# MatchaChoco010/toy-cpu-pathtracing

Measured on AMD Instinct MI355X. Metric: Msamples/sec (whole node), scene3 MIS/Sobol 1920x1080, higher is better.
Workload: dtype f32; 1 GPU; scene3 1920x1080 mis+sobol, 1024-spp job, 1024 sample indices per step (BASELINE configs[1]); parallelism=single-gpu

## Files before the change

### toy-cpu-pathtracing_amd/csrc/api.cpp

```cpp
#include <cstring>

#include "api_internal.hpp"

using namespace pt;

static thread_local std::string g_err;
bool pt::g_debug_unlocked = false;
int pt::fail(int code, const std::string& msg) { g_err = msg; return code; }

static const uint32_t CIE_CMF_BITS[470 * 4] = {
#include "cie_cmf.inc"
};
void pt::cie_cmf4(float out[470 * 4]) { std::memcpy(out, CIE_CMF_BITS, sizeof(CIE_CMF_BITS)); }

int pt::get_launch_ctx(const mi355pt_scene* sc, uint32_t seed, LaunchCtx** out, int* slot) {
    if (sc->ctx && sc->ctx->device != sc->impl.device) {
        delete sc->ctx; sc->ctx = nullptr;
    }
    if (!sc->ctx) {
        LaunchCtx* lc = new LaunchCtx();
        lc->device = sc->impl.device;
        HIP_TRY(hipMalloc((void**)&lc->d_hash, sizeof(uint64_t) * HASH_TABLE_DIMS));
        HIP_TRY(hipMalloc((void**)&lc->d_counters, sizeof(unsigned) * CTX_RING));
        HIP_TRY(hipMalloc((void**)&lc->d_stats, sizeof(DevStats) * CTX_RING));
// ... 88 lines not shown
    int rc;
    LaunchCtx* lc; int slot;
    if ((rc = get_launch_ctx(s, p->seed, &lc, &slot))) return rc;
    if (lc->device != s->impl.device) return fail(MI355PT_E_DEVICE, "launch context and scene live on different devices");
    const bool want_stats = stats && p->collect_stats;
    int& waves = aov ? lc->aov_waves[aov_kind] : lc->waves[want_stats ? 1 : 0][p->sampler & 1u][p->strategy < 3u ? p->strategy : 0u];
    if (!waves) waves = aov ? query_resident_waves_aov((uint32_t)aov_kind, s->impl.features)
                            : query_resident_waves(select_kernel(false, want_stats, s->impl.features, p->sampler, p->strategy));
    const DevCamera dc = make_camera(cam);
    LaunchPlan plan = d_list ? plan_launch_tiles(cam, p, s_begin, s_end, waves, n_list) : plan_launch(cam, p, s_begin, s_end, waves, aov);
    DevParams& dp = plan.params;
    if (d_list) set_tile_list(dp, d_list);
    dp.stats_mode = p->collect_stats;
    return timed_launch(lc, slot, stream, stats, want_stats || aov, [&](unsigned* d_counter, DevStats* d_stats) {
        if ((rc = grow_device_buffer(&lc->d_partial, &lc->partial_bytes, plan.partial_floats * sizeof(float), stream))) return rc;
        const KernelKey key = select_kernel(d_list != nullptr, want_stats, s->impl.features, p->sampler, p->strategy);
        if ((rc = grow_device_buffer(&lc->d_defer, &lc->defer_bytes, aov ? (size_t)0 : query_defer_bytes_per_wave(key) * (size_t)plan.grid, stream))) return rc;
        if (aov) HIP_TRY(launch_aov((uint32_t)aov_kind, s->impl.dev, dc, dp, illuminant_lut, lc->d_hash, d_accum, d_counter, stats ? d_stats : nullptr,
                                    s->impl.features, plan.grid, stream));
        else {
            DevScene dev = s->impl.dev;
            dev.cam_lists = use_camera_lists(key, dp.block_log2, camera_lists_enabled()) ? 1u : 0u;
            dev.queue_stage = use_queue_staging(key, queue_staging_enabled()) ? 1u : 0u;
            HIP_TRY(launch_pt(key, dev, dc, dp, plan.n_tiles,
                              lc->d_hash, d_accum, lc->d_partial, d_counter, d_list ? nullptr : d_stats, plan.grid, stream, pout, lc->d_defer));
        }
        return (int)MI355PT_OK;
    });
}

int pt::launch_ranges(const mi355pt_scene* s, const mi355pt_camera* cam, const mi355pt_params* p, uint32_t s_begin, uint32_t s_end, float* d_accum,
                      hipStream_t stream, mi355pt_stats* stats, const uint32_t* d_list, uint32_t n_list, const PathOut& pout, int aov_kind,
                      uint32_t illuminant_lut) {
    return for_each_launch_range(p->sampler, stats != nullptr, s_begin, s_end, [&](uint32_t b, uint32_t e) {
        return launch_range(s, cam, p, b, e, d_accum, stream, stats, pout, aov_kind, illuminant_lut, d_list, n_list);
    });
}

int pt::render_accum_range(const mi355pt_scene* s, const mi355pt_camera* cam, const mi355pt_params* p, uint32_t s_begin, uint32_t s_end,
                           float* d_accum, void* hip_stream, mi355pt_stats* stats, const PathOut& pout, int aov_kind, uint32_t illuminant_lut) {
    const bool aov = aov_kind >= 0;
    int rc = check_args(s, cam, p, aov);
    if (rc) return rc;
    if (!d_accum || s_end > p->spp || s_begin >= s_end) return fail(MI355PT_E_INVALID, "bad sample range or null accumulator");
    if (aov) {
        if (aov_kind > MI355PT_AOV_SHADING_NORMAL) return fail(MI355PT_E_INVALID, "unknown AOV kind");
// ... 97 lines not shown
```

### toy-cpu-pathtracing_amd/csrc/launch_plan.hpp

```cpp
#pragma once
#include <algorithm>
#include <cmath>
#include <cstddef>
#include <cstdint>
#include <cstdlib>

#include "../../include/mi355pt.h"
#include "layout.hpp"

namespace pt {

struct V3 { float x, y, z; };
inline V3 cross3(V3 a, V3 b) { return {a.y * b.z - b.y * a.z, a.z * b.x - b.z * a.x, a.x * b.y - b.x * a.y}; }
inline V3 norm3(V3 a) { float r = 1.0f / std::sqrt((a.x * a.x) + (a.y * a.y) + (a.z * a.z)); return {a.x * r, a.y * r, a.z * r}; }

inline uint32_t log2_int(uint32_t v) { return v == 0 ? 0 : 31 - (uint32_t)__builtin_clz(v); }
inline uint32_t round_up_pow2(uint32_t v) { return v <= 1 ? 1 : 1u << (32 - __builtin_clz(v - 1)); }

inline uint32_t shard_tile_count(uint32_t width, uint32_t height, uint32_t shard_index, uint32_t shard_count) {
    const uint32_t total = ((width + 7) / 8) * ((height + 7) / 8);
    const uint32_t cnt = shard_count ? shard_count : 1u, idx = shard_count ? shard_index : 0u;
    return total > idx ? (total - idx + cnt - 1) / cnt : 0u;
}

// ... 133 lines not shown
inline constexpr uint32_t FEATURE_SETS[] = {PT_FOR_EACH_SET(PT_SET_ENTRY, PT_SET_ENTRY)};
inline constexpr uint32_t PLAIN_SETS[] = {PT_FOR_EACH_PLAIN_SET(PT_SET_ENTRY)};
inline constexpr uint32_t CC_SETS[] = {PT_FOR_EACH_CC_SET(PT_SET_ENTRY)};
#undef PT_SET_ENTRY
inline uint32_t pick_features(uint32_t feat) {
    for (uint32_t s : FEATURE_SETS) if ((feat & ~s) == 0u) return s;
    return FEAT_ALL;
}
struct KernelKey { bool tiles, stats; uint32_t mode, set; };
inline KernelKey select_kernel(bool tiles, bool stats, uint32_t feat, uint32_t sampler, uint32_t strategy) {
    if (stats) return KernelKey{tiles, true, MODE_GENERIC, (feat & (FEAT_CC | FEAT_EMTEX)) == 0u ? FEAT_STD & ~FEAT_CC : FEAT_ALL};
    const uint32_t mode = sampler == MI355PT_SAMPLER_SOBOL && strategy == MI355PT_STRATEGY_MIS ? MODE_MIS_SOBOL
                        : sampler == MI355PT_SAMPLER_SOBOL && strategy == MI355PT_STRATEGY_NEE ? MODE_NEE_SOBOL
                        : strategy == MI355PT_STRATEGY_PT ? MODE_PT : MODE_GENERIC;
    return KernelKey{tiles, false, mode, pick_features(feat)};
}

inline bool use_camera_lists(const KernelKey& key, uint32_t block_log2, bool enabled) { return enabled && !key.stats && block_log2 <= 3u; }
inline bool camera_lists_enabled() { const char* e = getenv("MI355PT_NO_CAMERA_LISTS"); return !(e && e[0] != '\0' && !(e[0] == '0' && e[1] == '\0')); }

inline bool use_queue_staging(const KernelKey& key, bool enabled) { return enabled && !key.stats; }
inline bool queue_staging_enabled() { const char* e = getenv("MI355PT_NO_QUEUE_STAGING"); return !(e && e[0] != '\0' && !(e[0] == '0' && e[1] == '\0')); }

}
```

### toy-cpu-pathtracing_amd/csrc/layout.hpp

```cpp
#pragma once
#include <stddef.h>
#include <stdint.h>

#if defined(__HIPCC__)
#define PT_HD __host__ __device__
#else
#define PT_HD
#endif

namespace pt {

#ifndef PT_STACK_DEPTH
#define PT_STACK_DEPTH 24
#endif
constexpr int STACK_DEPTH = PT_STACK_DEPTH;
constexpr int MAX_LEAF_TRIS = 4;
constexpr int MAX_BUILD_DEPTH = 22;
constexpr int HASH_TABLE_DIMS = 136;

struct alignas(16) DevNode {
    float bx[4];
    float by[4];
    float bz[4];
    int32_t child[2];
// ... 138 lines not shown
    const DevTriLocal* tris_local;
    const DevTri* tris_render;
    float tri_shift[3]; uint32_t tris_are_local;
    float shared_mw[3]; uint32_t pad_mw;
    const DevInstance* instances;
    const DevMaterial* materials;
    const DevLight* lights;
    const DevLightTri* light_tris;
    const float* light_uvs;
    const float* luts;
    const float* cmf;
    const float* rgb2spec;
    const float* z_nodes;
    const uint32_t* texels;
    const DevTexture* textures;
    const float* cc_albedo;
    uint32_t n_nodes, n_tris, n_lights, n_materials;
    int32_t root;
    int32_t root4;
    uint32_t n_nodes4;
    uint32_t cam_lists;
    const DevEnv* envs;
    uint32_t n_envs;
    uint32_t queue_stage;
};

struct DevCamera {
    float s[3], u[3], f[3];
    float tan_half_fov, aspect;
    uint32_t width, height;
};

struct DevParams {
    uint32_t spp, seed, max_depth, strategy, sampler;
    float exposure;
    uint32_t log2_spp, n_base4_digits;
    uint32_t sample_begin, sample_end;
    uint32_t shard_index, shard_count;
    uint32_t tiles_x, tiles_y;
    uint32_t n_work;
    uint32_t chunks, chunk_size;
    uint32_t block_log2;
    uint32_t sample_prefix_digits;
    uint32_t stats_mode;
    uint32_t albedo_lut;
    float rr_gate;
    float xyz_to_rgb[9];
// ... 21 lines not shown
```

### toy-cpu-pathtracing_amd/csrc/pt_kernel.hpp

```cpp
#pragma once
#include <hip/hip_runtime.h>

#include "launch.hpp"
#include "launch_plan.hpp"
#include "layout.hpp"
#include "pt_device.hpp"
#include "pt_path.hpp"
#include "tail_queue_plan.hpp"
#define PT_CAM_UNIFORM(v) ((uint32_t)__builtin_amdgcn_readfirstlane((int)(v)))
#include "camera_candidates.hpp"

namespace pt {

constexpr uint32_t CAM_LIST_NONE = 0xffffffffu;

#ifndef PT_MIN_WAVES_CC
#define PT_MIN_WAVES_CC 3
#endif
#ifndef PT_MIN_WAVES
#define PT_MIN_WAVES 4
#endif
struct LaneJob { uint32_t px, py, s_cur, s_end; bool valid; };
template <typename TileOf>
PT_DEV LaneJob lane_job_at(uint32_t work, uint32_t lane, const DevCamera& cam, const DevParams& prm, TileOf tile_of) {
// ... 47 lines not shown
constexpr uint32_t DEFER_F4 = 8u;
constexpr uint32_t defer_classes_of(uint32_t FEAT, uint32_t MODE) {
    if (!merged_traversal_of(FEAT, MODE)) return 0u;
    if ((FEAT & FEAT_CC) != 0u) return (1u << MT_CLEARCOAT) | (1u << (MT_CLEARCOAT | 8u));
    if ((FEAT & FEAT_TEX) != 0u) return 0xff00u;
    return 0u;
}
template <uint32_t FEAT, uint32_t MODE> constexpr uint32_t defer_classes() { return defer_classes_of(FEAT, MODE); }
#ifndef PT_TAILQ
#define PT_TAILQ 1
#endif
#ifndef PT_TAILQ_MIN
#define PT_TAILQ_MIN 64
#endif
constexpr bool tail_queue_of(uint32_t FEAT, uint32_t MODE) { return PT_TAILQ != 0 && merged_traversal_of(FEAT, MODE); }
template <uint32_t FEAT, uint32_t MODE> constexpr bool tail_queue() { return tail_queue_of(FEAT, MODE); }
constexpr uint32_t QUEUE_RING = (PT_TAILQ != 0) ? 256u : DEFER_RING;
constexpr uint32_t QUEUE_MAX = (PT_TAILQ != 0) ? 2u : 1u;
static_assert(PT_TAILQ == 0 || QUEUE_RING == 256u, "the tail queue's entry index keeps the queue number in bit 8");
constexpr uint32_t TQ_F4 = 5u;
#ifndef PT_TAILQ_RING1
#define PT_TAILQ_RING1 128u
#endif
constexpr size_t queue_bytes_per_wave(bool STATS, uint32_t FEAT, uint32_t MODE) {
    if (!STATS && tail_queue_of(FEAT, MODE)) return (size_t)16u * TQ_F4 * ((FEAT & FEAT_CC) != 0u ? QUEUE_MAX * QUEUE_RING : PT_TAILQ_RING1);
    return defer_classes_of(FEAT, MODE) != 0u ? (size_t)16u * DEFER_F4 * DEFER_RING : (size_t)0;
}
template <uint32_t FEAT> constexpr int kernel_min_waves() {
    if ((FEAT & FEAT_CC) == 0u) return PT_MIN_WAVES;
    if (FEAT != (FEAT_CC | FEAT_TEX)) return 4;
    return PT_MIN_WAVES_CC;
}
template <bool STATS, uint32_t FEAT, uint32_t MODE = MODE_GENERIC>
__global__ __launch_bounds__(64, kernel_min_waves<FEAT>()) void pt_kernel(DevScene sc, DevCamera cam, DevParams prm_in, const uint64_t* __restrict__ dim_hash_tab,
                                                float* __restrict__ accum, float* __restrict__ partial, unsigned* __restrict__ work_counter,
                                                DevStats* __restrict__ stats, PathOut pout, float4* __restrict__ defer_buf) {
#define PT_LANE_JOB lane_job
#include "pt_kernel_body.inc"
#undef PT_LANE_JOB
}

PT_DEV void item_sobol_prefixes(SamplerCtx& sctx, const DevParams& prm, const LaneJob& job0, uint32_t lane, uint32_t* s_hi, uint32_t* s_p6, uint32_t n_dims) {
    const uint32_t blk_log2 = prm.block_log2;
    const uint32_t s_prefix = prm.sample_prefix_digits;
    const uint32_t hi_first_w = sobol_hi_first(prm.log2_spp, blk_log2) - s_prefix, hi_shift_w = 2u * hi_first_w - (prm.log2_spp & 1u);
    if (prm.sampler == 1u && hi_first_w < prm.n_base4_digits && hi_first_w >= 3u &&
        2u * prm.n_base4_digits - (prm.log2_spp & 1u) <= hi_shift_w + 27u) {
        sctx.hi_first = sobol_hi_first(prm.log2_spp, blk_log2) - s_prefix;
// ... 28 lines not shown
```

### toy-cpu-pathtracing_amd/csrc/pt_kernel_body.inc

```
    __shared__ __attribute__((aligned(16))) uint32_t s_stack[STACK_DEPTH * 64];
#ifndef PT_FILM_PIX
#define PT_FILM_PIX 64
#endif
    __shared__ float s_film[PT_FILM_PIX * 3];
    __shared__ uint32_t s_hi[SOBOL_HI_DIMS];
    __shared__ uint32_t s_p6[SOBOL_HI_DIMS];
    __shared__ unsigned s_work;
    constexpr bool PARK = (FEAT & FEAT_CC) != 0u && kernel_min_waves<FEAT>() <= 3;
    __shared__ float s_park[PARK ? 8 * 64 : 1];
    __shared__ uint8_t s_perm[96];
    __shared__ uint32_t s_ring[ANY_RING];
    __shared__ uint32_t s_occl[2];
    __shared__ uint32_t s_pair[64];
    const AnyLds any_lds{s_ring, s_occl, s_pair};
    __shared__ unsigned long long s_best[64];
    const ClosestLds closest_lds{s_ring, s_best, s_pair};
    __shared__ uint32_t s_infl[2];
    const PairLds pair_lds{s_ring, s_best, s_occl, s_pair, s_infl};
    constexpr bool CAMLIST = !STATS && tail_queue<FEAT, MODE>();
    __shared__ uint32_t s_cand[CAMLIST ? CAM_LIST_CAP : 1u];
    DevParams prm = prm_in;
    if constexpr (MODE == MODE_MIS_SOBOL) { prm.strategy = 2u; prm.sampler = 1u; }
    if constexpr (MODE == MODE_NEE_SOBOL) { prm.strategy = 1u; prm.sampler = 1u; }
    if constexpr (MODE == MODE_PT) prm.strategy = 0u;
// ... 65 lines not shown
        if (lane < PT_FILM_PIX) { s_film[3 * lane] = 0.0f; s_film[3 * lane + 1] = 0.0f; s_film[3 * lane + 2] = 0.0f; }
        __syncthreads();
        const uint32_t n_s = job0.s_end > job0.s_cur ? job0.s_end - job0.s_cur : 0u;
        const uint32_t pool_size = n_s << (2u * blk_log2);
        uint32_t pool_next = 0u;
        uint32_t my_pix = lane;
        Path P{};
        park(P);
        bool active = false;
        constexpr bool MERGED = merged_traversal<FEAT, MODE>();
        ShadowReq sh{};
        bool dying = false, susp = false;
        CarryState carry{0ull};
        constexpr bool TAILQ = !STATS && tail_queue<FEAT, MODE>();
        constexpr uint32_t DEFER = TAILQ ? 0u : defer_classes<FEAT, MODE>();
        float4* const q_base = (DEFER != 0u || TAILQ) ? defer_buf + (size_t)blockIdx.x * (queue_bytes_per_wave(STATS, FEAT, MODE) / 16u) : nullptr;
        uint32_t q_head = 0u, q_tail = 0u;
        uint32_t q_count = 0u, q2_count = 0u;
        constexpr uint32_t TQ_CLASSES = (TAILQ && (FEAT & FEAT_CC) != 0u) ? ((1u << MT_CLEARCOAT) | (1u << (MT_CLEARCOAT | 8u))) : 0u;
        constexpr uint32_t QR = (TQ_CLASSES != 0u) ? QUEUE_RING : PT_TAILQ_RING1;
        constexpr bool STAGE = TAILQ && TQ_CLASSES == 0u;
        static_assert(STACK_DEPTH * 64 >= (int)(TQ_STAGE_SLOTS * TQ_F4 * 4u) && TQ_STAGE_SLOTS == 64u, "a pass's worth of staged tail-queue records fits the traversal stack's LDS");
        float4* const s_stage = (float4*)s_stack;
        while (true) {
            unsigned long long ts0 = 0, ts1 = 0, ts2 = 0, ts3 = 0, ts4 = 0, tsa = 0, tsb = 0;
            uint32_t bsdf_classes = 0u;
            if (STATS) ts0 = __builtin_amdgcn_s_memtime();
            bool popped = false;
            uint32_t pop_e = 0u;
            const unsigned long long m_needy = __ballot(!active);
            if (m_needy != 0ull && pool_next < pool_size) {
                const uint32_t idx = pool_next + rank_below(m_needy);
                if (!active && idx < pool_size) {
                    const uint32_t pix = idx & ((1u << (2u * blk_log2)) - 1u);
                    const uint32_t px = job0.px + (pix & blk_mask), py = job0.py + (pix >> blk_log2);
                    const uint32_t smp_i = job0.s_cur + (idx >> (2u * blk_log2));
                    const bool valid = px < cam.width && py < cam.height;
                    if (valid) { active = true; my_pix = pix; regen_path<STATS>(P, sctx, cam, px, py, smp_i, st); }
                }
                pool_next = min(pool_next + (uint32_t)__popcll(m_needy), pool_size);
            }
            if (!__any(active)) {
                if (pool_next >= pool_size && q_tail == q_head && (q_count | q2_count) == 0u) break;
                if (!((DEFER != 0u || TAILQ) && pool_next >= pool_size)) continue;
            }
            if (STATS) { ts1 = __builtin_amdgcn_s_memtime(); if (lane == 0) st.w[4]++; if (active) st.w[5]++; }
            Hit hit{};
            bool got = false;
            const bool canonical = STATS && prm.stats_mode == 1u;
            if (canonical) { if (active) got = trace_closest<STATS>(sc, P.ro, P.rd, 3.402823466e+38f, stack, hit, st); }
            else if constexpr (MERGED) {
                bool occluded = false;
                if (STATS && sh.on) st.w[6]++;
                bool cam_ray = false;
                if constexpr (CAMLIST) cam_ray = cam_n != CAM_LIST_NONE && active && !dying && P.from_camera && P.depth == 0u;
                if (!CAMLIST || __ballot((active && !dying && !popped && !cam_ray) || sh.on) != 0ull) {
                    PT_PRIO_TRAV_ENTER;
                    trace_pair_coop<STATS>(sc, P.ro, P.rd, active && !dying && !popped && !cam_ray, sh.o, sh.d, sh.t, sh.on, stack, lane, pair_lds, hit, got, occluded, st, &carry, susp, &susp);
                    PT_PRIO_TRAV_EXIT;
                }
                if constexpr (CAMLIST) {
                    if (__ballot(cam_ray) != 0ull) {
                        const RaySetup rs = setup_ray(P.rd);
                        const f3 o2 = tri_origin(sc, P.ro);
                        unsigned long long key = (0x7f7fffffull << 32) | 0xffffffffull;
                        for (uint32_t i = 0u; i < cam_n; ++i) {
// ... 76 lines not shown
                const uint32_t fl = __float_as_uint(b.y);
                Q.smp.morton = __float_as_uint(a.x); Q.smp.dimension = __float_as_uint(a.y); Q.smp.rkey_lo = __float_as_uint(a.z); Q.smp.rkey_hi = __float_as_uint(a.w);
                Q.wl.lam0 = b.x; Q.wl.term = (fl & 1u) != 0u; Q.from_camera = (fl & 2u) != 0u; Q.prev_spec = (fl & 4u) != 0u; Q.depth = (fl >> 3) & 1023u; pix = fl >> 16;
                Q.T[0] = b.z; Q.T[1] = b.w; Q.T[2] = c.x; Q.T[3] = c.y; Q.L[0] = c.z; Q.L[1] = c.w; Q.L[2] = d.x; Q.L[3] = d.y;
                Q.rd = mk3(d.z, d.w, e4.x); Q.ro = mk3(0.0f, 0.0f, 0.0f);
                Q.pf[0] = e4.y; Q.pf[1] = e4.z; Q.pf[2] = e4.w; Q.pf[3] = f.x; Q.p_pdf = f.y; Q.prev_pos = mk3(f.z, f.w, g.x);
                h.t = g.y; h.b0 = g.z; h.b1 = g.w; h.b2 = h4.x; h.tri = __float_as_uint(h4.y); h.mclass = __float_as_uint(h4.z);
            };
            auto finish_path = [&]() {
                if (pout.L != nullptr) {
                    const uint32_t px = job0.px + (my_pix & blk_mask), py = job0.py + (my_pix >> blk_log2);
                    const uint32_t tile_k = (work / prm.chunks) >> (6u - 2u * blk_log2);
                    const uint32_t smp_i = P.smp.morton & ((1u << prm.log2_spp) - 1u);
                    sample_log(P, pout, ((size_t)tile_k * 64u + ((py & 7u) * 8u + (px & 7u))) * pout.n_s + (smp_i - pout.s_base));
                }
                float r, g, b;
                film_rgb(P, sc, prm, r, g, b);
                atomicAdd(&s_film[3 * my_pix], r); atomicAdd(&s_film[3 * my_pix + 1], g); atomicAdd(&s_film[3 * my_pix + 2], b);
            };
            if constexpr (TAILQ) {
                bool end_path = dying;
                const bool front = active && !dying && !susp;
                unpark(P);
                {
                    ShadeCtx C0;
                    C0.cont = false;
                    if (front) end_path = shade_vertex_head<STATS, FEAT, 1>(P, sc, prm, sctx, got, hit, sh, st, tsa, C0);
                }
                dying = false;
                const bool go_on = front && !end_path;
                const bool cls2 = TQ_CLASSES != 0u && ((TQ_CLASSES >> (hit.mclass & 31u)) & 1u) != 0u;
                const unsigned long long m_on1 = __ballot(go_on && !cls2), m_on2 = TQ_CLASSES != 0u ? __ballot(go_on && cls2) : 0ull;
                uint32_t n_on1 = 0u;
                bool stage = false;
                if constexpr (STAGE) {
                    n_on1 = (uint32_t)__popcll(m_on1);
                    stage = sc.queue_stage != 0u && tq_stage_pushes(q_count, n_on1, pool_next >= pool_size, (uint32_t)PT_TAILQ_MIN);
                }
                if ((m_on1 | m_on2) != 0ull) {
                    if (go_on) {
                        if (STAGE && stage) tq_put(s_stage + tq_stage_push_index(rank_below(m_on1)), TQ_STAGE_SLOTS, P, hit, my_pix);
                        else {
                            const uint32_t e = cls2 ? QUEUE_RING + tq_push_slot(q2_count, rank_below(m_on2)) : tq_push_slot(q_count, rank_below(m_on1));
                            tq_store(e, P, hit, my_pix);
                        }
                        active = false;
                    }
                    q_count += (uint32_t)__popcll(m_on1); q2_count += (uint32_t)__popcll(m_on2);
                    __builtin_amdgcn_fence(__ATOMIC_RELEASE, "workgroup");
                }
                if (active && end_path) { finish_path(); active = false; }
                park(P, false);
                if (STATS) ts3 = ts4 = __builtin_amdgcn_s_memtime();
                const bool draining = pool_next >= pool_size;
                if (tq_pass_due(q_count, q2_count, draining, TQ_CLASSES != 0u, (uint32_t)PT_TAILQ_MIN)) {
                    const unsigned long long m_free = __ballot(!active);
                    const uint32_t n_free = (uint32_t)__popcll(m_free), r = rank_below(m_free);
                    const TqTake tk = tq_pass_take(q_count, q2_count, n_free, draining, TQ_CLASSES != 0u, (uint32_t)PT_TAILQ_MIN);
                    const uint32_t n2 = tk.n2, n1 = tk.n1;
                    const bool take2 = !active && r < n2, take1 = !active && !take2 && r - n2 < n1;
                    const bool take = take1 || take2;
                    const uint32_t e = take2 ? QUEUE_RING + tq_pop_slot(q2_count, n2, r) : tq_pop_slot(q_count, n1, r - n2);
                    TqStagePop sp{0u, false, 0u};
                    if constexpr (STAGE) sp = tq_stage_pop(stage ? q_count - n_on1 : q_count, stage ? n_on1 : 0u, n1, r - n2);
                    q2_count -= n2; q_count -= n1;
                    bool ep = false;
                    if constexpr ((FEAT & FEAT_CC) != 0u) {
                        ShadeCtx C;
                        shade_ctx_idle_cc(C);
                        if (take) {
                            __builtin_amdgcn_fence(__ATOMIC_ACQUIRE, "workgroup");
                            tq_load(e, P, hit, my_pix);
                            active = true;
                            shade_vertex_head<STATS, FEAT, 2>(P, sc, prm, sctx, true, hit, sh, st, tsa, C);
                        }
// ... 140 lines not shown
```

### toy-cpu-pathtracing_amd/csrc/pt_path.hpp

```cpp
#pragma once
#include "launch.hpp"
#include "pt_device.hpp"
#include "pt_ggx.hpp"

namespace pt {

constexpr float RAY_EPS = 1e-5f;
constexpr float SHADOW_EPS = 1e-4f;

struct Frame { f3 t, b, n; };
PT_DEV f3 to_local(const Frame& f, f3 v) { return mk3(dot(f.t, v), dot(f.b, v), dot(f.n, v)); }
PT_DEV f3 to_world(const Frame& f, f3 v) { return f.t * v.x + f.b * v.y + f.n * v.z; }
PT_DEV Frame shading_frame(f3 shading_normal, f3 tangent) {
    Frame f;
    f.n = normalize(shading_normal);
    f.b = normalize(cross(normalize(f.n), tangent));
    f.t = normalize(cross(f.b, f.n));
    return f;
}
#ifndef PT_EXACT_DIV
#define PT_EXACT_DIV 0
#endif
#ifndef PT_FRAME_INVERSE
#define PT_FRAME_INVERSE 2
// ... 218 lines not shown
    float dx = (2.0f * fx / (float)cam.width - 1.0f) * cam.aspect * cam.tan_half_fov;
    float dy = (1.0f - 2.0f * fy / (float)cam.height) * cam.tan_half_fov;
    f3 dc = normalize(mk3(dx, dy, -1.0f));
    f3 s = mk3(cam.s[0], cam.s[1], cam.s[2]), uu = mk3(cam.u[0], cam.u[1], cam.u[2]), ff = mk3(cam.f[0], cam.f[1], cam.f[2]);
    rd = normalize(s * dc.x + uu * dc.y + (-ff) * dc.z);
    ro = mk3(0, 0, 0) + rd * RAY_EPS;
#pragma unroll
    for (int i = 0; i < 4; ++i) { T[i] = 1.0f; L[i] = 0.0f; }
    from_camera = true; depth = 0; need_new = false;
    if (STATS) st.samples++;
    (void)need_new;
}

PT_DEV f3 camera_ray_dir(const DevCamera& cam, uint32_t px, uint32_t py, f2 uv) {
    float fx = (float)px + (uv.x * 1.0f - 1.0f * 0.5f) + 0.5f;
    float fy = (float)py + (uv.y * 1.0f - 1.0f * 0.5f) + 0.5f;
    float dx = (2.0f * fx / (float)cam.width - 1.0f) * cam.aspect * cam.tan_half_fov;
    float dy = (1.0f - 2.0f * fy / (float)cam.height) * cam.tan_half_fov;
    f3 dc = normalize(mk3(dx, dy, -1.0f));
    f3 s = mk3(cam.s[0], cam.s[1], cam.s[2]), uu = mk3(cam.u[0], cam.u[1], cam.u[2]), ff = mk3(cam.f[0], cam.f[1], cam.f[2]);
    return normalize(s * dc.x + uu * dc.y + (-ff) * dc.z);
}

struct ShadeCtx {
    Surface sf; const DevMaterial* mat; uint32_t mtype;
    Frame fr, fw, nf, nfw; f3 wo, wo_nm, ng_t; float geo_wo, uc; f2 uv;
    bool is_diel, rough_diel, cont;
    float d_alpha;
    bool need_cc; float cc_alpha_c, cc_r0c, cc_thick, cc_metallic, cc_rough_b, cc_fc; uint64_t mc_key;
};

PT_DEV void shade_ctx_idle_cc(ShadeCtx& C) {
    C.cont = false; C.need_cc = false; C.cc_fc = 0.0f; C.cc_alpha_c = 0.0f; C.cc_r0c = 0.0f; C.wo_nm = mk3(0, 0, 1); C.mc_key = 0ull;
}

template <bool STATS, uint32_t FEAT, int PHASE = 0>
PT_DEV bool shade_vertex_head(Path& P, const DevScene& sc, const DevParams& prm, const SamplerCtx& sctx, bool got, const Hit& hit, ShadowReq& sh,
                           StatCounters& st, unsigned long long& tsa, ShadeCtx& C) {
    Sampler& smp = P.smp; Wl& wl = P.wl; float* T = P.T; float* L = P.L; f3& ro = P.ro; f3& rd = P.rd;
    bool& from_camera = P.from_camera; bool& prev_spec = P.prev_spec; float* pf = P.pf; float& p_pdf = P.p_pdf; f3& prev_pos = P.prev_pos;
    uint32_t& depth = P.depth;
    bool end_path = false;
    bool& do_shadow = sh.on; f3& sh_o = sh.o; f3& sh_d = sh.d; float& sh_t = sh.t; float* sh_c = sh.c;
    do_shadow = false;

    if (PHASE != 2 && !got) {
// ... 26 lines not shown
                    }
                    for (uint32_t li = 0; li < sc.n_lights; ++li) {
                        DevLight lt = sc.lights[li];
                        if (lt.kind != LK_ENV) continue;
                        const DevMaterial* lm = sc.materials + lt.material;
                        float ph[4];
                        DevSpectrum ls = load_spectrum(&lm->color);
                        eval_spectrum<false, (FEAT & FEAT_EMTEX) != 0, (FEAT & FEAT_EMTEX) != 0>(sc, ls, wl, f2{0.5f, 0.5f}, ph, st);
                        float sum = 0.0f;
#pragma unroll
                        for (int i = 0; i < 4; ++i) sum += (ph[i] * lm->intensity_avg) * lt.area_sum;
                        const float probability = inf_sum == 0.0f ? 0.0f : (sum / 4.0f) / inf_sum;
                        light_pdf += probability * env_pdf(sc.envs[lt.first_tri], rd);
                    }
                }
                float w = balance_heuristic(p_pdf, light_pdf);
                float tf = 1.0f / p_pdf;
#pragma unroll
                for (int i = 0; i < 4; ++i) L[i] = L[i] + ((((T[i] * pf[i]) * rad[i]) * tf) * w);
            }
        }
    } else {
        Surface sf; const DevMaterial* mat = nullptr; uint32_t mtype;
        if (PHASE == 1) {
            mtype = hit.mclass & 7u;
            if (mtype == MT_EMISSIVE) { sf = load_surface(sc, hit, rd); mat = sc.materials + sf.material; }
        } else { sf = load_surface(sc, hit, rd); mat = sc.materials + sf.material; mtype = mat->type; }
        const bool emissive = PHASE != 2 && mtype == MT_EMISSIVE;
        float Le[4] = {0, 0, 0, 0};
        if constexpr (PHASE != 2) {
        if (emissive) {
            DevSpectrum rs = load_spectrum(&mat->color);
            eval_spectrum<STATS, (FEAT & FEAT_EMTEX) != 0, (FEAT & FEAT_EMTEX) != 0>(sc, rs, wl, sf.uv, Le, st);
            float inten = mat->intensity;
            if ((FEAT & FEAT_EMTEX) && mat->metallic_tex != 0xffffffffu) { float t3[3]; bilinear_rgb(sc, mat->metallic_tex, sf.uv, t3); inten = t3[0]; }
#pragma unroll
            for (int i = 0; i < 4; ++i) Le[i] = Le[i] * inten;
        }
        if (from_camera) {
            if (emissive) {
#pragma unroll
                for (int i = 0; i < 4; ++i) L[i] = L[i] + T[i] * Le[i];
            }
        } else {
            float tf = 1.0f / p_pdf;
            if (emissive) {
                float w = 1.0f;
                if (prm.strategy == 1u) w = prev_spec ? 1.0f : 0.0f;
                else if (prm.strategy == 2u && !prev_spec) {
                    float wsum = 0.0f, wme = 0.0f;
                    if (!(FEAT & FEAT_MLIGHT) || sc.n_lights == 1u) {
// ... 39 lines not shown
            } else if (prm.strategy != 1u || prev_spec) {
                float w = (prm.strategy == 2u && !prev_spec) ? balance_heuristic(p_pdf, 0.0f) : 1.0f;
#pragma unroll
                for (int i = 0; i < 4; ++i) L[i] = L[i] + (T[i] * 0.0f) * w;
            }
#pragma unroll
            for (int i = 0; i < 4; ++i) T[i] = T[i] * (pf[i] * tf);
            float p = fmaxf(fmaxf(fmaxf(fmaxf(-INFINITY, T[0]), T[1]), T[2]), T[3]);
            if (!(p >= prm.rr_gate)) {
                float ur = get_1d(smp, sctx);
                if (ur < p) {
                    if (p != 0.0f) {
#pragma unroll
                        for (int i = 0; i < 4; ++i) T[i] = T[i] / p;
                    }
                } else end_path = true;
            }
        }
        if (!end_path) {
            depth += 1;
            if (depth > prm.max_depth || emissive) end_path = true;
        }
        }
        if (PHASE != 1 && !end_path) {
            if (STATS) { st.bounces++; tsa = __builtin_amdgcn_s_memtime(); }
            Frame fr, fw_num;
            if constexpr (numeric_frames<FEAT>()) shading_frames_numeric(sf.ns, sf.tangent, fr, fw_num);
            else fr = shading_frame(sf.ns, sf.tangent);
            const Frame& fw = numeric_frames<FEAT>() ? fw_num : fr;
            f3 wo_r = sf.wo;
            f3 wo = to_local(fr, wo_r);
            f3 ng_t = normalize(to_local(fw, sf.ng));
            const bool is_diel = (FEAT & FEAT_DIEL) && (mtype == MT_GLASS || mtype == MT_PLASTIC);
            float uc = 0.0f;
            f2 uv = f2{0.0f, 0.0f};
            float d_alpha = mat->roughness;
            if ((FEAT & FEAT_TEX) && (FEAT & FEAT_ROUGH) && is_diel && mat->roughness_tex != 0xffffffffu) { float t3[3]; bilinear_rgb(sc, mat->roughness_tex, sf.uv, t3); d_alpha = t3[0]; }
            const bool rough_diel = (FEAT & FEAT_ROUGH) && is_diel && d_alpha >= 1e-3f;
            if (is_diel) {
                uc = get_1d(smp, sctx);
                if (rough_diel || (mtype == MT_PLASTIC && mat->color.kind == SPK_TEXTURE)) uv = get_2d(smp, sctx); else smp.dimension += 2;
            }
            else if ((FEAT & FEAT_CC) && mtype == MT_CLEARCOAT) { uc = get_1d(smp, sctx); uv = get_2d(smp, sctx); }
            else { smp.dimension += 1; uv = get_2d(smp, sctx); }
            Frame nf, nfw_num;
            if ((FEAT & FEAT_TEX) && mat->normal_tex != 0xffffffffu) {
                float rgb[3];
// ... 627 lines not shown
```

### toy-cpu-pathtracing_amd/csrc/scene_lower.cpp

```cpp
#include "scene_lower.hpp"

#include <algorithm>
#include <cfloat>
#include <cmath>
#include <cstdio>
#include <cstring>

#include "instance_move_plan.hpp"

namespace pt {

namespace {

constexpr float PI_F = 3.14159265358979323846f;

struct V3 { float x, y, z; };
inline V3 operator-(V3 a, V3 b) { return {a.x - b.x, a.y - b.y, a.z - b.z}; }
inline V3 cross(V3 a, V3 b) { return {a.y * b.z - b.y * a.z, a.z * b.x - b.z * a.x, a.x * b.y - b.x * a.y}; }
inline float dot(V3 a, V3 b) { return (a.x * b.x) + (a.y * b.y) + (a.z * b.z); }
inline float length(V3 a) { return std::sqrt(dot(a, a)); }
inline V3 normalize(V3 a) { float r = 1.0f / length(a); return {a.x * r, a.y * r, a.z * r}; }
inline V3 vertex(const HostMesh& mesh, uint32_t v) { return V3{mesh.pos[3 * v], mesh.pos[3 * v + 1], mesh.pos[3 * v + 2]}; }
inline bool degenerate(V3 a, V3 b, V3 c) { const V3 cr = cross(b - a, c - a); return dot(cr, cr) == 0.0f; }

// ... 674 lines not shown
           " depth=" + std::to_string(rep.bvh_depth) + " builder=" + (gpu_builder ? "gpu" : "host") + t_bvh + " collapse=" + rep.collapse_method + t_collapse + tail;
}

void lowering_digests(const LoweredScene& ls, const LowerReport& rep, std::vector<std::string>* names, std::vector<uint64_t>* digests) {
    names->clear(); digests->clear();
    auto add = [&](const std::string& name, const void* p, size_t bytes) { names->push_back(name); digests->push_back(fnv1a64(p, bytes)); };
#define PT_DIGEST(v) add(#v, ls.v.data(), ls.v.size() * sizeof(ls.v[0]))
    PT_DIGEST(nodes); PT_DIGEST(nodes4); PT_DIGEST(tris_render); PT_DIGEST(shade); PT_DIGEST(instances); PT_DIGEST(tris_local); PT_DIGEST(cc_albedo);
    PT_DIGEST(materials); PT_DIGEST(lights); PT_DIGEST(light_tris); PT_DIGEST(light_uvs); PT_DIGEST(luts); PT_DIGEST(cmf); PT_DIGEST(rgb2spec);
    PT_DIGEST(z_nodes); PT_DIGEST(texels); PT_DIGEST(textures);
#undef PT_DIGEST
    for (size_t k = 0; k < ls.env_tables.size(); ++k) {
        const LoweredScene::EnvTables& t = ls.env_tables[k];
        const std::string e = "env" + std::to_string(k);
        add(e + ".texels", t.texels.data(), t.texels.size() * 4); add(e + ".marginal", t.marginal.data(), t.marginal.size() * 4);
        add(e + ".conditional", t.conditional.data(), t.conditional.size() * 4);
    }
    add("envs", ls.envs.data(), ls.envs.size() * sizeof(DevEnv));
    std::string b;
    auto put = [&](const void* p, size_t n) { b.append((const char*)p, n); };
    const DevScene& dev = ls.dev;
    put(dev.grid_org, 12); put(dev.grid_cell, 12); put(dev.tri_shift, 12); put(&dev.tris_are_local, 4); put(dev.shared_mw, 12); put(&dev.pad_mw, 4);
    put(&dev.n_nodes, 4); put(&dev.n_tris, 4); put(&dev.n_lights, 4); put(&dev.n_materials, 4); put(&dev.root, 4); put(&dev.root4, 4);
    put(&dev.n_nodes4, 4); put(&dev.cam_lists, 4); put(&dev.n_envs, 4); put(&dev.queue_stage, 4);
    const uint32_t feat = ls.features; const uint64_t ndeg = rep.n_degenerate, nn4 = dev.n_nodes4; const int32_t depth = rep.bvh_depth, need = rep.stack_need;
    put(&feat, 4); put(&ndeg, 8); put(&depth, 4); put(&nn4, 8); put(&need, 4); put(rep.collapse_method, std::strlen(rep.collapse_method));
    add("scalars", b.data(), b.size());
}

}
```

### toy-cpu-pathtracing_amd/csrc/tail_queue_plan.hpp

```cpp
#pragma once
#include <cstdint>

namespace pt {

constexpr uint32_t tq_push_slot(uint32_t count, uint32_t rank) { return count + rank; }
constexpr uint32_t tq_pop_slot(uint32_t count, uint32_t n, uint32_t rank) { return count - n + rank; }

struct TqTake { uint32_t n1, n2; };

constexpr bool tq_pass_due(uint32_t c1, uint32_t c2, bool draining, bool two_queues, uint32_t pass_min) {
    return (two_queues && c2 >= pass_min) || c1 >= pass_min || (draining && (c1 | c2) != 0u);
}
constexpr TqTake tq_pass_take(uint32_t c1, uint32_t c2, uint32_t n_free, bool draining, bool two_queues, uint32_t pass_min) {
    const bool full2 = two_queues && c2 >= pass_min, full1 = c1 >= pass_min;
    const uint32_t n2 = (full2 || (draining && !full1)) ? (n_free < c2 ? n_free : c2) : 0u;
    const uint32_t n1 = (!full2 || draining) ? (n_free - n2 < c1 ? n_free - n2 : c1) : 0u;
    return TqTake{n1, n2};
}

constexpr uint32_t TQ_STAGE_SLOTS = 64u;

constexpr bool tq_stage_pushes(uint32_t count, uint32_t n_push, bool draining, uint32_t pass_min) {
    return n_push != 0u && tq_pass_due(count + n_push, 0u, draining, false, pass_min);
}
constexpr uint32_t tq_stage_push_index(uint32_t rank) { return rank; }

struct TqStagePop { uint32_t slot; bool staged; uint32_t index; };
constexpr TqStagePop tq_stage_pop(uint32_t count, uint32_t n_push, uint32_t n_take, uint32_t rank) {
    const uint32_t slot = tq_pop_slot(count + n_push, n_take, rank);
    return TqStagePop{slot, slot >= count, slot >= count ? slot - count : 0u};
}

}
```

Baseline: 2749 Msamples/s.

## Defer emitter-hit shading into a per-wave light queue processed in full-wave passes

Paths whose ray hits an emissive surface are no longer shaded in place. Their state is written to a per-wave ring in global scratch, and the emitter contribution is evaluated later in batches of up to 64 lanes, which is meant to cut SIMD divergence from scattered emitter hits. The head shading phase gains a PHASE 3 variant that skips emissive handling, and the DevScene queue_stage field is split into two 16-bit fields to carry an env-var toggle. The cost is extra global traffic for the 7-float4 records, a larger defer buffer, and added control flow and register pressure in the main loop.

```diff
diff --git a/toy-cpu-pathtracing_amd/csrc/api.cpp b/toy-cpu-pathtracing_amd/csrc/api.cpp
--- a/toy-cpu-pathtracing_amd/csrc/api.cpp
+++ b/toy-cpu-pathtracing_amd/csrc/api.cpp
@@ -134,6 +134,7 @@
             DevScene dev = s->impl.dev;
             dev.cam_lists = use_camera_lists(key, dp.block_log2, camera_lists_enabled()) ? 1u : 0u;
             dev.queue_stage = use_queue_staging(key, queue_staging_enabled()) ? 1u : 0u;
+            dev.light_queue = use_light_queue(key, light_queue_enabled()) ? 1u : 0u;
             HIP_TRY(launch_pt(key, dev, dc, dp, plan.n_tiles,
                               lc->d_hash, d_accum, lc->d_partial, d_counter, d_list ? nullptr : d_stats, plan.grid, stream, pout, lc->d_defer));
         }
diff --git a/toy-cpu-pathtracing_amd/csrc/launch_plan.hpp b/toy-cpu-pathtracing_amd/csrc/launch_plan.hpp
--- a/toy-cpu-pathtracing_amd/csrc/launch_plan.hpp
+++ b/toy-cpu-pathtracing_amd/csrc/launch_plan.hpp
@@ -179,4 +179,7 @@
 inline bool use_queue_staging(const KernelKey& key, bool enabled) { return enabled && !key.stats; }
 inline bool queue_staging_enabled() { const char* e = getenv("MI355PT_NO_QUEUE_STAGING"); return !(e && e[0] != '\0' && !(e[0] == '0' && e[1] == '\0')); }
 
+inline bool use_light_queue(const KernelKey& key, bool enabled) { return enabled && !key.stats; }
+inline bool light_queue_enabled() { const char* e = getenv("MI355PT_NO_LIGHT_QUEUE"); return !(e && e[0] != '\0' && !(e[0] == '0' && e[1] == '\0')); }
+
 }
diff --git a/toy-cpu-pathtracing_amd/csrc/layout.hpp b/toy-cpu-pathtracing_amd/csrc/layout.hpp
--- a/toy-cpu-pathtracing_amd/csrc/layout.hpp
+++ b/toy-cpu-pathtracing_amd/csrc/layout.hpp
@@ -184,7 +184,8 @@
     uint32_t cam_lists;
     const DevEnv* envs;
     uint32_t n_envs;
-    uint32_t queue_stage;
+    uint16_t queue_stage;
+    uint16_t light_queue;
 };
 
 struct DevCamera {
diff --git a/toy-cpu-pathtracing_amd/csrc/pt_kernel.hpp b/toy-cpu-pathtracing_amd/csrc/pt_kernel.hpp
--- a/toy-cpu-pathtracing_amd/csrc/pt_kernel.hpp
+++ b/toy-cpu-pathtracing_amd/csrc/pt_kernel.hpp
@@ -93,8 +93,10 @@
 #ifndef PT_TAILQ_RING1
 #define PT_TAILQ_RING1 128u
 #endif
+constexpr uint32_t LQ_F4 = 7u;
+constexpr bool light_queue_of(uint32_t FEAT, uint32_t MODE) { return tail_queue_of(FEAT, MODE) && (FEAT & FEAT_CC) == 0u; }
 constexpr size_t queue_bytes_per_wave(bool STATS, uint32_t FEAT, uint32_t MODE) {
-    if (!STATS && tail_queue_of(FEAT, MODE)) return (size_t)16u * TQ_F4 * ((FEAT & FEAT_CC) != 0u ? QUEUE_MAX * QUEUE_RING : PT_TAILQ_RING1);
+    if (!STATS && tail_queue_of(FEAT, MODE)) return (size_t)16u * TQ_F4 * ((FEAT & FEAT_CC) != 0u ? QUEUE_MAX * QUEUE_RING : PT_TAILQ_RING1) + (light_queue_of(FEAT, MODE) ? (size_t)16u * LQ_F4 * LQ_SLOTS : (size_t)0);
     return defer_classes_of(FEAT, MODE) != 0u ? (size_t)16u * DEFER_F4 * DEFER_RING : (size_t)0;
 }
 template <uint32_t FEAT> constexpr int kernel_min_waves() {
diff --git a/toy-cpu-pathtracing_amd/csrc/pt_kernel_body.inc b/toy-cpu-pathtracing_amd/csrc/pt_kernel_body.inc
--- a/toy-cpu-pathtracing_amd/csrc/pt_kernel_body.inc
+++ b/toy-cpu-pathtracing_amd/csrc/pt_kernel_body.inc
@@ -111,6 +111,19 @@
         constexpr bool STAGE = TAILQ && TQ_CLASSES == 0u;
         static_assert(STACK_DEPTH * 64 >= (int)(TQ_STAGE_SLOTS * TQ_F4 * 4u) && TQ_STAGE_SLOTS == 64u, "a pass's worth of staged tail-queue records fits the traversal stack's LDS");
         float4* const s_stage = (float4*)s_stack;
+        constexpr bool LIGHTQ = STAGE && light_queue_of(FEAT, MODE);
+        float4* const lq_base = LIGHTQ ? q_base + TQ_F4 * PT_TAILQ_RING1 : nullptr;
+        uint32_t lq_count = 0u;
+        auto lq_put = [&](float4* r, const Path& Q, const Hit& h, uint32_t pix) {
+            const uint32_t fl = (Q.wl.term ? 1u : 0u) | (Q.from_camera ? 2u : 0u) | (Q.prev_spec ? 4u : 0u) | ((pix & 63u) << 3);
+            r[0u * LQ_SLOTS] = make_float4(__uint_as_float(Q.smp.morton), __uint_as_float(fl), Q.wl.lam0, __uint_as_float(h.tri));
+            r[1u * LQ_SLOTS] = make_float4(Q.T[0], Q.T[1], Q.T[2], Q.T[3]);
+            r[2u * LQ_SLOTS] = make_float4(Q.L[0], Q.L[1], Q.L[2], Q.L[3]);
+            r[3u * LQ_SLOTS] = make_float4(Q.pf[0], Q.pf[1], Q.pf[2], Q.pf[3]);
+            r[4u * LQ_SLOTS] = make_float4(Q.rd.x, Q.rd.y, Q.rd.z, Q.p_pdf);
+            r[5u * LQ_SLOTS] = make_float4(Q.prev_pos.x, Q.prev_pos.y, Q.prev_pos.z, h.b0);
+            r[6u * LQ_SLOTS] = make_float4(h.b1, h.b2, 0.0f, 0.0f);
+        };
         while (true) {
             unsigned long long ts0 = 0, ts1 = 0, ts2 = 0, ts3 = 0, ts4 = 0, tsa = 0, tsb = 0;
             uint32_t bsdf_classes = 0u;
@@ -130,7 +143,7 @@
                 pool_next = min(pool_next + (uint32_t)__popcll(m_needy), pool_size);
             }
             if (!__any(active)) {
-                if (pool_next >= pool_size && q_tail == q_head && (q_count | q2_count) == 0u) break;
+                if (pool_next >= pool_size && q_tail == q_head && (q_count | q2_count | lq_count) == 0u) break;
                 if (!((DEFER != 0u || TAILQ) && pool_next >= pool_size)) continue;
             }
             if (STATS) { ts1 = __builtin_amdgcn_s_memtime(); if (lane == 0) st.w[4]++; if (active) st.w[5]++; }
@@ -253,13 +266,25 @@
                 bool end_path = dying;
                 const bool front = active && !dying && !susp;
                 unpark(P);
+                bool lq_push = false, lq_void = false;
+                if constexpr (LIGHTQ) {
+                    const bool on_emitter = front && got && (hit.mclass & 7u) == MT_EMISSIVE;
+                    lq_void = on_emitter && emitter_hit_is_void<STATS>(prm, P.from_camera, P.prev_spec);
+                    lq_push = on_emitter && !lq_void;
+                }
+                const unsigned long long m_lq = (LIGHTQ && sc.light_queue != 0u) ? __ballot(lq_push) : 0ull;
                 {
                     ShadeCtx C0;
                     C0.cont = false;
-                    if (front) end_path = shade_vertex_head<STATS, FEAT, 1>(P, sc, prm, sctx, got, hit, sh, st, tsa, C0);
+                    if constexpr (LIGHTQ) {
+                        if (front && !lq_push && !lq_void) end_path = shade_vertex_head<STATS, FEAT, 3>(P, sc, prm, sctx, got, hit, sh, st, tsa, C0);
+                        if (lq_void) end_path = true;
+                    } else {
+                        if (front) end_path = shade_vertex_head<STATS, FEAT, 1>(P, sc, prm, sctx, got, hit, sh, st, tsa, C0);
+                    }
                 }
                 dying = false;
-                const bool go_on = front && !end_path;
+                const bool go_on = front && !lq_push && !end_path;
                 const bool cls2 = TQ_CLASSES != 0u && ((TQ_CLASSES >> (hit.mclass & 31u)) & 1u) != 0u;
                 const unsigned long long m_on1 = __ballot(go_on && !cls2), m_on2 = TQ_CLASSES != 0u ? __ballot(go_on && cls2) : 0ull;
                 uint32_t n_on1 = 0u;
@@ -268,7 +293,14 @@
                     n_on1 = (uint32_t)__popcll(m_on1);
                     stage = sc.queue_stage != 0u && tq_stage_pushes(q_count, n_on1, pool_next >= pool_size, (uint32_t)PT_TAILQ_MIN);
                 }
-                if ((m_on1 | m_on2) != 0ull) {
+                if ((m_on1 | m_on2 | m_lq) != 0ull) {
+                    if constexpr (LIGHTQ) {
+                        if (lq_push && m_lq != 0ull) {
+                            lq_put(lq_base + (lq_push_slot(lq_count, rank_below(m_lq)) & (LQ_SLOTS - 1u)), P, hit, my_pix);
+                            active = false;
+                        }
+                        lq_count += (uint32_t)__popcll(m_lq);
+                    }
                     if (go_on) {
                         if (STAGE && stage) tq_put(s_stage + tq_stage_push_index(rank_below(m_on1)), TQ_STAGE_SLOTS, P, hit, my_pix);
                         else {
@@ -282,6 +314,34 @@
                 }
                 if (active && end_path) { finish_path(); active = false; }
                 park(P, false);
+                if constexpr (LIGHTQ) {
+                    bool ev = lq_push;
+                    if (sc.light_queue != 0u) {
+                        ev = false;
+                        if (lq_pass_due(lq_count, pool_next >= pool_size && q_count == 0u)) {
+                            const uint32_t n = lq_pass_take(lq_count);
+                            ev = lane < n;
+                            if (ev) {
+                                __builtin_amdgcn_fence(__ATOMIC_ACQUIRE, "workgroup");
+                                const float4* r = lq_base + (lq_pop_slot(lq_count, n, lane) & (LQ_SLOTS - 1u));
+                                const float4 a = r[0u * LQ_SLOTS], b = r[1u * LQ_SLOTS], c = r[2u * LQ_SLOTS], d = r[3u * LQ_SLOTS], e4 = r[4u * LQ_SLOTS], f = r[5u * LQ_SLOTS], g = r[6u * LQ_SLOTS];
+                                const uint32_t fl = __float_as_uint(a.y);
+                                P.smp.morton = __float_as_uint(a.x); P.wl.lam0 = a.z; P.wl.term = (fl & 1u) != 0u;
+                                P.from_camera = (fl & 2u) != 0u; P.prev_spec = (fl & 4u) != 0u; my_pix = (fl >> 3) & 63u;
+                                P.T[0] = b.x; P.T[1] = b.y; P.T[2] = b.z; P.T[3] = b.w; P.L[0] = c.x; P.L[1] = c.y; P.L[2] = c.z; P.L[3] = c.w;
+                                P.pf[0] = d.x; P.pf[1] = d.y; P.pf[2] = d.z; P.pf[3] = d.w;
+                                P.rd = mk3(e4.x, e4.y, e4.z); P.p_pdf = e4.w; P.prev_pos = mk3(f.x, f.y, f.z);
+                                hit.b0 = f.w; hit.b1 = g.x; hit.b2 = g.y; hit.tri = __float_as_uint(a.w);
+                            }
+                            lq_count -= n;
+                        }
+                    }
+                    if (ev) {
+                        emitter_hit<STATS, FEAT>(sc, prm, hit, P.rd, P.T, P.pf, P.p_pdf, P.prev_pos, P.wl, P.from_camera, P.prev_spec, P.L, st);
+                        finish_path();
+                        active = false;
+                    }
+                }
                 if (STATS) ts3 = ts4 = __builtin_amdgcn_s_memtime();
                 const bool draining = pool_next >= pool_size;
                 if (tq_pass_due(q_count, q2_count, draining, TQ_CLASSES != 0u, (uint32_t)PT_TAILQ_MIN)) {
diff --git a/toy-cpu-pathtracing_amd/csrc/pt_path.hpp b/toy-cpu-pathtracing_amd/csrc/pt_path.hpp
--- a/toy-cpu-pathtracing_amd/csrc/pt_path.hpp
+++ b/toy-cpu-pathtracing_amd/csrc/pt_path.hpp
@@ -264,6 +264,80 @@
     return normalize(s * dc.x + uu * dc.y + (-ff) * dc.z);
 }
 
+template <bool STATS>
+PT_DEV bool emitter_hit_is_void(const DevParams& prm, bool from_camera, bool prev_spec) {
+    return !STATS && prm.strategy == 1u && !from_camera && !prev_spec;
+}
+template <bool STATS, uint32_t FEAT>
+PT_DEV void emitter_contribution(const DevScene& sc, const DevParams& prm, const Surface& sf, const DevMaterial* mat, const float* T, const float* pf,
+                                 float p_pdf, f3 prev_pos, const Wl& wl, bool from_camera, bool prev_spec, float* L, StatCounters& st) {
+    if (emitter_hit_is_void<STATS>(prm, from_camera, prev_spec)) return;
+    float Le[4] = {0, 0, 0, 0};
+    DevSpectrum rs = load_spectrum(&mat->color);
+    eval_spectrum<STATS, (FEAT & FEAT_EMTEX) != 0, (FEAT & FEAT_EMTEX) != 0>(sc, rs, wl, sf.uv, Le, st);
+    float inten = mat->intensity;
+    if ((FEAT & FEAT_EMTEX) && mat->metallic_tex != 0xffffffffu) { float t3[3]; bilinear_rgb(sc, mat->metallic_tex, sf.uv, t3); inten = t3[0]; }
+#pragma unroll
+    for (int i = 0; i < 4; ++i) Le[i] = Le[i] * inten;
+    if (from_camera) {
+#pragma unroll
+        for (int i = 0; i < 4; ++i) L[i] = L[i] + T[i] * Le[i];
+        return;
+    }
+    float tf = 1.0f / p_pdf;
+    float w = 1.0f;
+    if (prm.strategy == 1u) w = prev_spec ? 1.0f : 0.0f;
+    else if (prm.strategy == 2u && !prev_spec) {
+        float wsum = 0.0f, wme = 0.0f;
+        if (!(FEAT & FEAT_MLIGHT) || sc.n_lights == 1u) {
+            float sum = 0.0f;
+            float area = sc.lights[0].area_sum;
+            if ((FEAT & FEAT_EMTEX) && (mat->color.kind == SPK_TEXTURE || mat->metallic_tex != 0xffffffffu)) {
+                float ph[4];
+                DevSpectrum ls = load_spectrum(&mat->color);
+                eval_spectrum<false, true, true>(sc, ls, wl, f2{0.5f, 0.5f}, ph, st);
+#pragma unroll
+                for (int i = 0; i < 4; ++i) sum += (ph[i] * mat->intensity_avg) * area;
+            } else {
+#pragma unroll
+                for (int i = 0; i < 4; ++i) sum += Le[i] * area;
+            }
+            wsum = wme = sum / 4.0f;
+        } else
+        for (uint32_t li = 0; li < sc.n_lights; ++li) {
+            DevLight lt = sc.lights[li];
+            const DevMaterial* lm = sc.materials + lt.material;
+            float ph[4];
+            DevSpectrum ls = load_spectrum(&lm->color);
+            eval_spectrum<false, (FEAT & FEAT_EMTEX) != 0, (FEAT & FEAT_EMTEX) != 0>(sc, ls, wl, f2{0.5f, 0.5f}, ph, st);
+            float inten_l = lm->intensity_avg;
+            float sum = 0.0f;
+#pragma unroll
+            for (int i = 0; i < 4; ++i) sum += (ph[i] * inten_l) * lt.area_sum;
+            float wt = sum / 4.0f;
+            wsum += wt;
+            if (li == sf.light) wme = wt;
+        }
+        float probability = wsum == 0.0f ? 0.0f : wme / wsum;
+        f3 dv = prev_pos - sf.p;
+        float distance = length(dv);
+        f3 wo_l = -normalize(dv);
+        float pdf_dir = sf.light_pdf_area * (distance * distance) / fabsf(dot(sf.ng, wo_l));
+        w = balance_heuristic(p_pdf, probability * pdf_dir);
+    }
+    if (w != 0.0f || prm.strategy != 1u) {
+#pragma unroll
+        for (int i = 0; i < 4; ++i) L[i] = L[i] + (T[i] * ((pf[i] * Le[i]) * tf)) * w;
+    }
+}
+template <bool STATS, uint32_t FEAT>
+PT_DEV void emitter_hit(const DevScene& sc, const DevParams& prm, const Hit& hit, f3 rd, const float* T, const float* pf, float p_pdf, f3 prev_pos,
+                        const Wl& wl, bool from_camera, bool prev_spec, float* L, StatCounters& st) {
+    if (emitter_hit_is_void<STATS>(prm, from_camera, prev_spec)) return;
+    const Surface sf = load_surface(sc, hit, rd);
+    emitter_contribution<STATS, FEAT>(sc, prm, sf, sc.materials + sf.material, T, pf, p_pdf, prev_pos, wl, from_camera, prev_spec, L, st);
+}
+
 struct ShadeCtx {
     Surface sf; const DevMaterial* mat; uint32_t mtype;
     Frame fr, fw, nf, nfw; f3 wo, wo_nm, ng_t; float geo_wo, uc; f2 uv;
@@ -336,11 +410,11 @@
         }
     } else {
         Surface sf; const DevMaterial* mat = nullptr; uint32_t mtype;
-        if (PHASE == 1) {
+        if (PHASE == 1 || PHASE == 3) {
             mtype = hit.mclass & 7u;
-            if (mtype == MT_EMISSIVE) { sf = load_surface(sc, hit, rd); mat = sc.materials + sf.material; }
+            if (PHASE == 1 && mtype == MT_EMISSIVE) { sf = load_surface(sc, hit, rd); mat = sc.materials + sf.material; }
         } else { sf = load_surface(sc, hit, rd); mat = sc.materials + sf.material; mtype = mat->type; }
-        const bool emissive = PHASE != 2 && mtype == MT_EMISSIVE;
+        const bool emissive = PHASE != 2 && PHASE != 3 && mtype == MT_EMISSIVE;
         float Le[4] = {0, 0, 0, 0};
         if constexpr (PHASE != 2) {
         if (emissive) {
@@ -426,7 +500,7 @@
             if (depth > prm.max_depth || emissive) end_path = true;
         }
         }
-        if (PHASE != 1 && !end_path) {
+        if (PHASE != 1 && PHASE != 3 && !end_path) {
             if (STATS) { st.bounces++; tsa = __builtin_amdgcn_s_memtime(); }
             Frame fr, fw_num;
             if constexpr (numeric_frames<FEAT>()) shading_frames_numeric(sf.ns, sf.tangent, fr, fw_num);
diff --git a/toy-cpu-pathtracing_amd/csrc/scene_lower.cpp b/toy-cpu-pathtracing_amd/csrc/scene_lower.cpp
--- a/toy-cpu-pathtracing_amd/csrc/scene_lower.cpp
+++ b/toy-cpu-pathtracing_amd/csrc/scene_lower.cpp
@@ -720,7 +720,7 @@
     const DevScene& dev = ls.dev;
     put(dev.grid_org, 12); put(dev.grid_cell, 12); put(dev.tri_shift, 12); put(&dev.tris_are_local, 4); put(dev.shared_mw, 12); put(&dev.pad_mw, 4);
     put(&dev.n_nodes, 4); put(&dev.n_tris, 4); put(&dev.n_lights, 4); put(&dev.n_materials, 4); put(&dev.root, 4); put(&dev.root4, 4);
-    put(&dev.n_nodes4, 4); put(&dev.cam_lists, 4); put(&dev.n_envs, 4); put(&dev.queue_stage, 4);
+    put(&dev.n_nodes4, 4); put(&dev.cam_lists, 4); put(&dev.n_envs, 4); put(&dev.queue_stage, 2); put(&dev.light_queue, 2);
     const uint32_t feat = ls.features; const uint64_t ndeg = rep.n_degenerate, nn4 = dev.n_nodes4; const int32_t depth = rep.bvh_depth, need = rep.stack_need;
     put(&feat, 4); put(&ndeg, 8); put(&depth, 4); put(&nn4, 8); put(&need, 4); put(rep.collapse_method, std::strlen(rep.collapse_method));
     add("scalars", b.data(), b.size());
diff --git a/toy-cpu-pathtracing_amd/csrc/tail_queue_plan.hpp b/toy-cpu-pathtracing_amd/csrc/tail_queue_plan.hpp
--- a/toy-cpu-pathtracing_amd/csrc/tail_queue_plan.hpp
+++ b/toy-cpu-pathtracing_amd/csrc/tail_queue_plan.hpp
@@ -31,4 +31,12 @@
     return TqStagePop{slot, slot >= count, slot >= count ? slot - count : 0u};
 }
 
+constexpr uint32_t LQ_SLOTS = 128u;
+constexpr uint32_t LQ_PASS = 64u;
+constexpr uint32_t LQ_MAX_WAITING = 127u;
+constexpr uint32_t lq_push_slot(uint32_t count, uint32_t rank) { return count + rank; }
+constexpr bool lq_pass_due(uint32_t count, bool item_done) { return count >= LQ_PASS || (item_done && count != 0u); }
+constexpr uint32_t lq_pass_take(uint32_t count) { return count < LQ_PASS ? count : LQ_PASS; }
+constexpr uint32_t lq_pop_slot(uint32_t count, uint32_t n, uint32_t rank) { return count - n + rank; }
+
 }
```

New measurement: 2799 Msamples/s (median of 6 runs). 1.8% higher.
